# worldfnd/provekit

Hardware: AMD Instinct MI355X
Metric: proofs/sec (noir-r1cs prove hot path, WHIR commit + sumcheck + folding rounds) (higher is better)
Workload: dtype u32x8 (BN254-Fr, 256-bit Montgomery integers); 1 GPU; poseidon-rounds size class: m=21, m_0=20, satisfiable synthetic R1CS (786429 constraints, 1048571 witnesses, a constant term in half of the rows of A and B), batch-2 WHIR commit + zk-sumcheck + 4-round WHIR opening, queries [109, 28, 16, 11]/9, pow_bits [19.0, 16.0, 16.0, 18.0]/11.0 (WhirConfig::new derivation, security 128, ConjectureList), blinding WHIR n=8 queries [122]/31, Skyscraper-sponge tr; launcher=single process

## Files before the change

provekit_amd/_lib.py:

```python
from __future__ import annotations

import ctypes as C
import os

_HERE = os.path.dirname(os.path.abspath(__file__))
LIB_PATH = os.environ.get("PK_LIB_PATH") or os.path.join(_HERE, "lib", "libprovekit_hip.so")

PK_OK = 0
PK_LEAF_MAJOR = 0
PK_COL_MAJOR = 1

_ERR_NAMES = {-1: "PK_ERR_BAD_ARG", -2: "PK_ERR_OOM", -3: "PK_ERR_HIP", -4: "PK_ERR_RCCL", -5: "PK_ERR_NO_DEVICE", -6: "PK_ERR_UNSATISFIED"}


class ProveKitHipError(RuntimeError):
    def __init__(self, code, msg):
        super().__init__(f"{_ERR_NAMES.get(code, code)}: {msg}")
        self.code = code


def _load():
    if not os.path.exists(LIB_PATH):
        raise ImportError(
            f"{LIB_PATH} is missing: build it with `python -c 'import __graft_entry__ as g; g.build()'` "
# ... 125 lines not shown
}


class WhirConfigStruct(C.Structure):
    _fields_ = [("n_vars", C.c_uint), ("batch_size", C.c_uint), ("folding_factor", C.c_uint), ("starting_log_inv_rate", C.c_uint),
                ("n_rounds", C.c_uint), ("num_queries", C.c_uint * 16), ("ood_samples", C.c_uint * 16), ("pow_bits", C.c_double * 16),
                ("final_queries", C.c_uint), ("final_pow_bits", C.c_double), ("commitment_ood_samples", C.c_uint),
                ("final_folding_pow_bits", C.c_double)]


class SparseMatrixStruct(C.Structure):
    _fields_ = [("new_row_indices", vp), ("col_indices", vp), ("values", vp), ("nnz", sz)]

SELFTEST_SIGNATURES = {
    "pk_selftest_set_host_tail": (C.c_int, [vp, C.c_uint]),
    "pk_selftest_eq_suffix_tables": (C.c_int, [vp, vp, C.c_uint, vp]),
    "pk_selftest_sumcheck_cubic_spliteq": (C.c_int, [vp, vp, vp, vp, vp, C.c_uint, C.c_uint, vp, vp, vp]),
    "pk_selftest_sumcheck_quadratic_claim": (C.c_int, [vp, vp, vp, sz, vp, vp, vp, vp, vp]),
    "pk_selftest_keccak_tag": (C.c_int, [vp, sz, vp]),
    "pk_selftest_permute": (C.c_int, [vp, vp]),
    "pk_selftest_arith": (C.c_int, [C.c_int, vp, vp, vp, sz]),
    "pk_selftest_chacha": (C.c_int, [vp, C.c_uint64, C.c_uint32, C.c_uint32, C.c_int, vp]),
    "pk_selftest_random_fe": (C.c_int, [vp, vp, C.c_uint32, vp, sz]),
    "pk_selftest_dft": (C.c_int, [vp, vp, vp, C.c_int, C.c_int, sz]),
    "pk_selftest_pre_load": (C.c_int, [vp, vp, vp, C.c_int, C.c_int, sz]),
    "pk_selftest_set_hook": (C.c_int, [C.c_int, C.c_long]),
}

for _name, (_res, _args) in list(SIGNATURES.items()) + list(SELFTEST_SIGNATURES.items()):
    if _name in SELFTEST_SIGNATURES and os.environ.get("PK_LIB_PATH") and not hasattr(lib, _name):
# ... 5 lines not shown
```

provekit_amd/csrc/ctx.hip:

```cpp
#include "internal.hpp"
#include "fe29.hpp"

#include <sys/prctl.h>
#include <time.h>

#include <atomic>

using namespace pk;

#define PK_MAX_DEVICES 64
static std::atomic<int> g_poll_wait[PK_MAX_DEVICES];
static std::atomic<long> g_test_hooks[pk::PK_HOOK_COUNT];
static std::atomic<int> g_runtime_wait[PK_MAX_DEVICES];
static const bool g_runtime_wait_init = [] {
    for (auto& w : g_runtime_wait) w.store(-1, std::memory_order_relaxed);
    return true;
}();

namespace pk {
long test_hook(int which) { return which >= 0 && which < PK_HOOK_COUNT ? g_test_hooks[which].load(std::memory_order_relaxed) : 0; }
hipError_t wait_stream(int device, hipStream_t stream) {
    if (device < 0 || device >= PK_MAX_DEVICES || !g_poll_wait[device].load(std::memory_order_relaxed)) return hipStreamSynchronize(stream);
    long slack = -1;
    hipError_t e;
// ... 246 lines not shown
}

int pk_ctx_set_latency_mode(pk_ctx* ctx, int on) {
    if (!ctx) return PK_ERR_BAD_ARG;
    ctx->latency_mode = on != 0;
    return PK_OK;
}

int pk_selftest_set_host_tail(pk_ctx* ctx, unsigned log2_len) {
    if (!ctx) return PK_ERR_BAD_ARG;
    if (log2_len > PK_HOST_TAIL_MAX_LOG2) return set_err(ctx, PK_ERR_BAD_ARG, "bad argument: host tail threshold is 0 (off) or 1 .. %d", PK_HOST_TAIL_MAX_LOG2);
    ctx->host_tail_log2 = log2_len;
    return PK_OK;
}

}

namespace pk {
int ensure_scratch(pk_ctx* ctx, size_t bytes) {
    if (ctx->scratch_bytes >= bytes) return PK_OK;
    if (ctx->d_scratch) {
        PK_WAIT(ctx);
        PK_HIP(ctx, hipFree(ctx->d_scratch));
        ctx->d_scratch = nullptr;
        ctx->scratch_bytes = 0;
    }
    size_t sz = bytes < (1u << 20) ? (1u << 20) : bytes;
    PK_HIP(ctx, hipMalloc(&ctx->d_scratch, sz));
    ctx->scratch_bytes = sz;
    ctx->red_armed = ctx->pow_armed = false;
// ... 83 lines not shown
```

provekit_amd/csrc/ctx.hpp:

```cpp
#pragma once
#include <hip/hip_runtime.h>

#include <cstdarg>
#include <cstdio>
#include <cstring>
#include <map>
#include <string>
#include <vector>

#include "../../include/provekit_hip.h"

struct pk_prof_rec {
    const char* name;
    hipEvent_t e0, e1;
};

struct pk_comm;

#ifndef PK_HOST_TAIL_DEFAULT_LOG2
#define PK_HOST_TAIL_DEFAULT_LOG2 10
#endif
#define PK_HOST_TAIL_MAX_LOG2 11

struct pk_ctx {
    int device = 0;
    pk_comm* comm = nullptr;
    bool prof_on = false;
    std::vector<pk_prof_rec> prof;
    std::vector<hipEvent_t> ev_pool;
    hipStream_t own_stream = nullptr;
    hipStream_t stream = nullptr;
    hipEvent_t ev_start = nullptr, ev_stop = nullptr;
    int hash_version = 2;
    int num_cus = 256;
    char err[512] = {0};
    int err_code = 0;
    void* d_scratch = nullptr;
    size_t scratch_bytes = 0;
    void* h_pinned = nullptr;
    size_t pinned_bytes = 0;
    std::map<unsigned long long, void*> tables;
    unsigned red_seq = 0;
    bool latency_mode = false;
    unsigned gate_seq = 0;
    unsigned host_tail_log2 = PK_HOST_TAIL_DEFAULT_LOG2;
    void* d_ws = nullptr;
    void* d_ztab = nullptr;
    size_t ws_bytes = 0;
    char* h_mail = nullptr;
    size_t mail_bytes = 0, mail_off = 0;
    bool pow_armed = false;
    bool red_armed = false;
    bool red_across = false;
    void* d_xred = nullptr;
    const void* red_scales = nullptr;
};
#define PK_XRED_OWN_BYTES 2048

#define PK_PIN_ROOT 2048
#define PK_PIN_POW 2112
// ... 96 lines not shown
```

provekit_amd/csrc/prover.hip:

```cpp
#include <unistd.h>

#include <algorithm>
#include <chrono>
#include <cstdlib>
#include <string>
#include <vector>

#include "host_tail.hpp"
#include "internal.hpp"
#include "shard_map.hpp"
#include "prover_transcript.hpp"

using namespace pk;

struct pk_scheme {
    const pk_r1cs* r1cs = nullptr;
    size_t num_constraints = 0, num_witnesses = 0;
    unsigned m = 0, m_0 = 0;
    unsigned nb = 0;
    pk_whir_config whir_witness{}, whir_hiding{};
    char* arena = nullptr;
    size_t arena_bytes = 0;
    std::string domain_separator;
    char* noir_witness = nullptr;
// ... 137 lines not shown
    }
    for (int i = 0; i < 4; i++) out[i] = c[i];
}

std::vector<uint64_t> stir_queries(Transcript& T, size_t domain_size, unsigned fold, unsigned num_queries) {
    std::vector<uint8_t> raw(stir_query_bytes(domain_size, fold) * num_queries);
    T.challenge_bytes(raw.data(), raw.size());
    return stir_indexes(raw.data(), domain_size, fold, num_queries);
}

int pow_round(pk_ctx* ctx, Transcript& T, double bits) {
    if (bits <= 0.0) return PK_OK;
    uint8_t challenge[POW_CHALLENGE_BYTES], be[POW_NONCE_BYTES];
    T.challenge_bytes(challenge, sizeof challenge);
    uint64_t nonce = 0;
    const int rc = pow_solve_x(ctx, challenge, bits, &nonce, comm_world(ctx) > 1);
    nonce_to_bytes(nonce, be);
    T.add_bytes(be, sizeof be);
    return rc;
}

struct Commitment {
    unsigned n_vars = 0, batch = 0;
    fe* polys[4] = {};
    fe* evals[4] = {};
    fe* leaves = nullptr;
    fe* nodes = nullptr;
    size_t rows = 0, width = 0;
    pk_commit_layout layout{};
    std::vector<fe> ood_points;
    std::vector<fe> ood_answers;
    fe beta;
};

int emit_opening_hints(pk_ctx* ctx, Transcript& T, const Commitment& C, const std::vector<uint64_t>& idx) {
    const size_t k = idx.size(), width = C.width;
    const unsigned logn = ilog2(C.rows);
    const size_t plen = logn ? logn - 1 : 0;
    std::vector<uint64_t> leaves(4 * k * width), sib(4 * (k ? k : 1)), paths(4 * (k * plen ? k * plen : 1));
    CK(open_raw(ctx, U(C.leaves), U(C.nodes), C.rows, width, C.layout, idx.data(), k, 1, leaves.data(), sib.data(), paths.data()));
    const auto ser0 = std::chrono::steady_clock::now();
    std::vector<uint8_t> buf;
    put_u64(buf, k);
    for (size_t q = 0; q < k; q++) put_vec(buf, (const fe*)(leaves.data() + 4 * q * width), width, false);
    T.hint(buf.data(), buf.size());
    size_t len = 0;
    pk_multipath_serialize(idx.data(), k, plen, sib.data(), paths.data(), nullptr, 0, &len);
    std::vector<uint8_t> mp(len ? len : 1);
    CK(pk_multipath_serialize(idx.data(), k, plen, sib.data(), paths.data(), mp.data(), len, &len));
    T.hint(mp.data(), len);
    T.hint_seconds += std::chrono::duration<double>(std::chrono::steady_clock::now() - ser0).count();
    return PK_OK;
}

int whir_commit_compute(pk_ctx* ctx, Arena& A, unsigned n_vars, unsigned log_inv_rate, unsigned fold, fe* const* polys, unsigned batch,
                        Commitment& C) {
    C.n_vars = n_vars;
    C.batch = batch;
    C.rows = (size_t)1 << (n_vars + log_inv_rate - fold);
    C.width = (size_t)batch << fold;
    for (unsigned b = 0; b < batch; b++) C.polys[b] = polys[b];
    ALLOC(leaves, C.rows * C.width / shard_factor(ctx, C.rows));
    ALLOC(nodes, 2 * C.rows);
    C.leaves = leaves;
    C.nodes = nodes;
    CK(ensure_ws(ctx, commit_scratch_fes(ctx, C.rows, C.width) * 32));
    const uint64_t* ptrs[4];
    for (unsigned b = 0; b < batch; b++) ptrs[b] = U(polys[b]);
    return commit_into(ctx, ptrs, batch, n_vars, log_inv_rate, fold, U(leaves), U(nodes), (uint64_t*)ctx->d_ws, &C.layout);
}
int whir_commit_transcript(pk_ctx* ctx, const pk_whir_config& cfg, const fe& root, Transcript& T, Commitment& C) {
    const unsigned batch = C.batch;
    fe* const* polys = C.polys;
    T.add_canon(root);
    C.ood_points.resize(cfg.commitment_ood_samples);
    T.challenge_scalars(C.ood_points.data(), C.ood_points.size());
    C.ood_answers.resize((size_t)batch * C.ood_points.size());
    for (size_t j = 0; j < C.ood_points.size(); j++) {
        for (unsigned b = 0; b < batch; b += 2) {
            const unsigned np = batch - b >= 2 ? 2 : 1;
            fe ans[2];
            CK(eval_univariate_multi_x(ctx, polys + b, np, (size_t)1 << cfg.n_vars, C.ood_points[j], ans));
            for (unsigned q = 0; q < np; q++) C.ood_answers[(b + q) * C.ood_points.size() + j] = ans[q];
        }
    }
    for (unsigned b = 0; b < batch; b++) T.add_scalars(&C.ood_answers[b * C.ood_points.size()], C.ood_points.size());
    C.beta = batch > 1 ? T.challenge_scalar() : fe_one();
    return PK_OK;
}

bool whir_sharded(const pk_ctx* ctx, unsigned n_vars) {
    const size_t G = (size_t)comm_world(ctx);
    return G > 1 && (((size_t)1 << n_vars) / G) >= 2 * SHARD_MIN_LOCAL;
}
size_t in_block(size_t stored, size_t off, size_t len) {
    const size_t hi = stored < off + len ? stored : off + len;
    return hi > off ? hi - off : 0;
// ... 64 lines not shown

struct WhirProver {
    pk_ctx* ctx;
    Arena& A;
    const pk_whir_config& cfg;
    const Commitment& C;
    Transcript& T;
    const unsigned n, k, G, lgG, rank;
    bool sharded;
    const size_t B0, off0;
    fe* d_c = nullptr;
    fe* bp[2] = {};
    fe* bw[2] = {};
    fe* gathered[4] = {};
    bool host = false;
    std::vector<fe> hp, hw;
    const fe* h_weight = nullptr;
    int cur = 0;
    size_t len;
    std::vector<fe> rs;
    fe claim;
    bool have_claim = false;
    std::vector<fe> all_r;

    WhirProver(pk_ctx* c, Arena& a, const pk_whir_config& cf, const Commitment& com, Transcript& t)
        : ctx(c), A(a), cfg(cf), C(com), T(t), n(cf.n_vars), k(cf.folding_factor), G((unsigned)comm_world(c)), lgG(ilog2(G)),
          rank((unsigned)comm_rank(c)), sharded(whir_sharded(c, n)), B0(sharded ? ((size_t)1 << n) / G : (size_t)1 << n),
          off0(sharded ? (size_t)rank * B0 : 0), len(B0) {}

    int batch_combine(fe* dst, fe* const* x, size_t from, size_t cnt) {
        if (C.batch == 1) return pk_memcpy_d2d(ctx, dst, x[0] + from, 32 * cnt);
// ... 135 lines not shown
        return PK_OK;
    }
    int maybe_gather() { return sharded && len <= SHARD_MIN_LOCAL ? gather(gathered[0], gathered[1], gathered[2], gathered[3]) : PK_OK; }

    int start(fe* const* d_weights, const size_t* weight_len, unsigned n_weights, const fe* weight_sums, const fe* h_evals, const fe* h_w) {
        const size_t N = (size_t)1 << n;
        if (h_evals) {
            PK_REQUIRE(ctx, !sharded && C.batch == 2 && n_weights <= 1 && (!n_weights || (h_w && weight_len[0] <= N)),
                       "an opening that starts on the host: batch 2, one weight");
            host = true;
            h_weight = h_w;
            hp.resize(N);
            hw.resize(N);
            host_tail::lincomb2(hp.data(), h_evals, C.beta, h_evals + N, N);
        }
        ALLOC(dc, N);
        d_c = dc;
        ALLOC(p0, B0);
        ALLOC(p1, B0 / 2 ? B0 / 2 : 1);
        ALLOC(w0, B0);
        ALLOC(w1, B0 / 2 ? B0 / 2 : 1);
        bp[0] = p0; bp[1] = p1; bw[0] = w0; bw[1] = w1;
        bool have_evals = true;
        for (unsigned b = 0; b < C.batch; b++) have_evals = have_evals && C.evals[b] != nullptr;
        const bool pair = have_evals && C.batch == 2;
        const bool rows3 = rows_at_equal_stride3(d_weights, weight_len, n_weights);
        const size_t tail = host_tail_len(ctx);
        const bool fused = !host && !(tail && !sharded && B0 <= tail) && pair && !sharded && B0 >= 2 && k >= 1 && (rows3 || n_weights == 1) && weight_len[0] <= B0;
        if (fused || host) {
            h_store(first.beta, C.beta);
            CK(lincomb2(ctx, U(d_c), U(C.polys[0]), first.beta, U(C.polys[1]), N));
        } else if (pair) {
            uint64_t s[4];
            h_store(s, C.beta);
            CK(lincomb2_pair(ctx, U(d_c), U(C.polys[0]), U(C.polys[1]), N, U(p0), U(C.evals[0] + off0), U(C.evals[1] + off0), B0, s));
        } else {
            CK(batch_combine(d_c, C.polys, 0, N));
        }
        if (host) {
        } else if (have_evals) {
            if (!pair) CK(batch_combine(p0, C.evals, off0, B0));
        } else if (!sharded) {
            CK(pk_to_evals_into(ctx, U(d_c), U(p0), n));
        } else {
// ... 48 lines not shown
                gathered[q] = buf;
            }
        }
        CK(sumcheck_rounds(k));
        return maybe_gather();
    }

    int rounds() {
        const Commitment* prev = &C;
        Commitment com;
        unsigned nv = n, log_inv_rate = cfg.starting_log_inv_rate;
        size_t domain_size = (size_t)1 << (n + log_inv_rate);
        fe exp_gen = folded_domain_generator(n + log_inv_rate, k);
        for (unsigned r = 0; r < cfg.n_rounds; r++) {
            const unsigned nv2 = nv - k;
            ALLOC(d_c2, (size_t)1 << nv2);
            CK(pk_fold_coeffs(ctx, U(d_c), nv, (const uint64_t*)rs.data(), k, U(d_c2)));
            d_c = d_c2;
            nv = nv2;
            log_inv_rate += k - 1;
            Commitment next;
            CK(whir_commit_compute(ctx, A, nv, log_inv_rate, k, &d_c, 1, next));
            fe root;
            CK(read_root(ctx, U(next.nodes), next.rows, (uint64_t*)root.v));
            T.add_canon(root);
            std::vector<fe> zs(cfg.ood_samples[r]);
            T.challenge_scalars(zs.data(), zs.size());
            std::vector<fe> ood_ans(zs.size());
            for (size_t j = 0; j < zs.size(); j++) CK(eval_univariate_x(ctx, d_c, (size_t)1 << nv, zs[j], ood_ans[j]));
            T.add_scalars(ood_ans.data(), ood_ans.size());
            CK(pow_round(ctx, T, cfg.pow_bits[r]));
            const std::vector<uint64_t> idx = stir_queries(T, domain_size, k, cfg.num_queries[r]);
            CK(emit_opening_hints(ctx, T, *prev, idx));
            const fe gamma = T.challenge_scalar();
            for (uint64_t i : idx) zs.push_back(h_pow(exp_gen, i));
            fe g;
            CK(maybe_to_host());
            CK(eq_weights(bw[cur], nv, zs, gamma, 0, &g, !host && !sharded && len >= 2 && k >= 1));
            have_claim = false;
            CK(sumcheck_rounds(k));
            CK(maybe_gather());
            com = next;
            prev = &com;
            domain_size /= 2;
            exp_gen = h_mul(exp_gen, exp_gen);
        }
        return final_round(*prev, nv, domain_size);
    }

    int final_round(const Commitment& prev, unsigned nv, size_t domain_size) {
        if (sharded) {
            const size_t cap = len * G;
            ALLOC(fp0, cap);
            ALLOC(fp1, cap / 2 ? cap / 2 : 1);
            ALLOC(fw0, cap);
            ALLOC(fw1, cap / 2 ? cap / 2 : 1);
            CK(gather(fp0, fp1, fw0, fw1));
        }
        const unsigned nv2 = nv - k;
        ALLOC(d_final, (size_t)1 << nv2);
        CK(pk_fold_coeffs(ctx, U(d_c), nv, (const uint64_t*)rs.data(), k, U(d_final)));
        std::vector<fe> fin((size_t)1 << nv2);
        CK(pk_memcpy_d2h(ctx, fin.data(), d_final, 32 * fin.size()));
        T.add_scalars(fin.data(), fin.size());
        CK(pow_round(ctx, T, cfg.final_pow_bits));
        const std::vector<uint64_t> idx = stir_queries(T, domain_size, k, cfg.final_queries);
        CK(emit_opening_hints(ctx, T, prev, idx));
        CK(sumcheck_rounds(nv2));
        return pow_round(ctx, T, cfg.final_folding_pow_bits);
    }

    int deferred_hint(fe* const* d_weights, const size_t* weight_len, unsigned n_weights) {
        if (!n_weights) return PK_OK;
        std::vector<fe> point(all_r.rbegin(), all_r.rend());
        const bool sh = whir_sharded(ctx, n);
        std::vector<fe> evals(n_weights);
        const bool rows3 = rows_at_equal_stride3(d_weights, weight_len, n_weights);
        if (h_weight) {
// ... 33 lines not shown
        return PK_OK;
    }
};
int whir_prove(pk_ctx* ctx, Arena& A, const pk_whir_config& cfg, const Commitment& C, fe* const* d_weights, const size_t* weight_len,
               unsigned n_weights, const fe* weight_sums, Transcript& T, const fe* h_evals = nullptr, const fe* h_weight = nullptr) {
    WhirProver P(ctx, A, cfg, C, T);
    CK(P.start(d_weights, weight_len, n_weights, weight_sums, h_evals, h_weight));
    CK(P.rounds());
    return P.deferred_hint(d_weights, weight_len, n_weights);
}

struct BatchCommit {
    Commitment com;
    fe* f_evals = nullptr;
    fe* g_evals = nullptr;
};
int batch_commit_compute(pk_ctx* ctx, Arena& A, unsigned m, const pk_whir_config& cfg, const fe* d_evals, size_t n_evals, const RngKey& key,
                         u32 stream_mask, u32 stream_g, BatchCommit& out) {
    const size_t half = (size_t)1 << (m - 1), N = 2 * half;
    ALLOC(f, N);
    ALLOC(g, N);
    ALLOC(fe_, N);
    ALLOC(ge_, N);
    if (comm_world(ctx) <= 1) {
        CK(to_coeffs_generated(ctx, m, U(d_evals), n_evals, key, stream_mask, stream_g, U(f), U(g), U(fe_), U(ge_)));
    } else {
        CK(pk_memset_zero(ctx, f, 32 * half));
        CK(pk_memcpy_d2d(ctx, f, d_evals, 32 * n_evals));
        {
            ProfScope prof(ctx, "random_fe");
// ... 79 lines not shown
    fe row_sums[6];
    const bool timing = getenv("PK_PROVE_TIMING") != nullptr;
    std::chrono::steady_clock::time_point t_lap = std::chrono::steady_clock::now();

    Proof(pk_ctx* c, pk_scheme* sc, const fe* w, size_t nw, const RngKey& k)
        : ctx(c), s(sc), d_witness(w), n_witness(nw), key(k), A{sc->arena, sc->arena_bytes}, T(sc->domain_separator), G((unsigned)comm_world(c)),
          lgG(ilog2(G)), rank((unsigned)comm_rank(c)), st_sharded(whir_sharded(c, sc->m)), blk(((size_t)1 << sc->m) / (st_sharded ? G : 1)),
          blk_lo(st_sharded ? (size_t)rank * blk : 0), aux(c), g_univ(4 * (size_t)sc->m_0) {}

    int init() {
        if (!ctx->latency_mode || G != 1) return PK_OK;
        CK(side.open(ctx, s));
        aux = side.c;
        return PK_OK;
    }
    pk_ctx* rows_ctx() const { return n_witness ? aux : ctx; }
    int relay(pk_ctx* c, int rc, const char* what) {
        if (!rc || c == ctx) return rc;
        return set_err(ctx, rc, "%s on the side stream: %s", what, pk_last_error(c));
    }
    void lap(const char* what) {
        if (!timing) return;
        (void)wait_ctx(ctx);
        const auto t = std::chrono::steady_clock::now();
        fprintf(stderr, "[pk_prove] %-28s %8.3f ms (sponge: %u permutes, %.3f ms; hint serialisation so far %.3f ms)\n", what,
                1e3 * std::chrono::duration<double>(t - t_lap).count(), T.permutes(), 1e3 * T.permute_seconds, 1e3 * T.hint_seconds);
        t_lap = t;
    }

    int commit_witness();
// ... 8 lines not shown
int blinding_compute(pk_ctx* ctx, Proof& P) {
    Arena& A = P.A;
    const size_t NB = (size_t)1 << P.s->nb, n = P.g_univ.size();
    ALLOC(d_blind, NB);
    CK(pk_memset_zero(ctx, d_blind, 32 * NB));
    CK(random_fe(ctx, U(d_blind), n, P.key, RNG_BLIND));
    if (ctx == P.ctx) {
        CK(pk_memcpy_d2h(ctx, P.g_univ.data(), d_blind, 32 * n));
    } else {
        CK(mail_alloc(ctx, 32 * n, (void**)&P.h_univ));
        PK_HIP(ctx, hipMemcpyAsync(P.h_univ, d_blind, 32 * n, hipMemcpyDeviceToHost, ctx->stream));
    }
    return batch_commit_compute(ctx, A, P.s->nb + 1, P.s->whir_hiding, d_blind, NB, P.key, RNG_MASK_B, RNG_G_B, P.B);
}

int external_rows(pk_ctx* ctx, Proof& P) {
    Arena& A = P.A;
    const size_t nw = P.n_witness;
    ALLOC(d_eq_alpha, (size_t)1 << P.s->m_0);
    ALLOC(rows, 3 * (nw ? nw : 1));
    P.rows = rows;
    CK(pk_eq_table(ctx, (const uint64_t*)P.alpha.data(), P.s->m_0, U(d_eq_alpha)));
    if (P.st_sharded) CK(external_row_range(ctx, P.s->r1cs, U(d_eq_alpha), P.blk_lo, std::min(nw, P.blk_lo + P.blk), U(rows)));
    else CK(pk_r1cs_external_row(ctx, P.s->r1cs, U(d_eq_alpha), U(rows)));
    if (ctx == P.ctx) return PK_OK;
    return dot_rows(ctx, U(rows), nw, 3, U(P.W.f_evals), U(P.W.g_evals), nw, nullptr, true);
}

int Proof::commit_witness() {
    CK(batch_commit_compute(ctx, A, s->m, s->whir_witness, d_witness, n_witness, key, RNG_MASK, RNG_G, W));
    if (aux != ctx) CK(relay(aux, blinding_compute(aux, *this), "blinding commitment"));
    fe root;
    CK(read_root(ctx, U(W.com.nodes), W.com.rows, (uint64_t*)root.v));
    return whir_commit_transcript(ctx, s->whir_witness, root, T, W.com);
}

int Proof::blinding_transcript() {
    fe root;
    CK(relay(aux, read_root(aux, U(B.com.nodes), B.com.rows, (uint64_t*)root.v), "blinding commitment"));
    if (h_univ) memcpy(g_univ.data(), h_univ, 32 * g_univ.size());
    return whir_commit_transcript(ctx, s->whir_hiding, root, T, B.com);
}

void zk_round_message(const uint64_t out[12], const fe gp[4], const fe& rho, const fe& saved, fe c[4]) {
    const fe half = h_half();
    c[0] = h_add(h_load(out), h_mul(rho, gp[0]));
    const fe g_m1 = h_sub(h_add(h_sub(gp[0], gp[1]), gp[2]), gp[3]);
    const fe at_m1 = h_add(h_load(out + 4), h_mul(rho, g_m1));
    c[2] = h_mul(half, h_sub(h_sub(h_sub(h_add(saved, at_m1), c[0]), c[0]), c[0]));
    c[3] = h_add(h_load(out + 8), h_mul(rho, gp[3]));
    c[1] = h_sub(h_sub(h_sub(h_sub(saved, c[0]), c[0]), c[3]), c[2]);
}

int Proof::zk_sumcheck() {
// ... 3 lines not shown
    const size_t M0 = (size_t)1 << m_0;
    const bool sharded = G > 1 && M0 / G >= 2 * SHARD_MIN_LOCAL;
    const size_t length = sharded ? M0 / G : M0;
    ALLOC(d_a, length);
    ALLOC(d_b, length);
    ALLOC(d_cc, length);
    ALLOC(d_eq, length);
    if (sharded) {
        CK(witness_bounds_strided(ctx, s->r1cs, U(d_witness), m_0, G, rank, U(d_a), U(d_b), U(d_cc)));
        const fe sc = eq_bits(&r[m_0 - lgG], lgG, rank);
        CK(pk_eq_accumulate(ctx, U(d_eq), m_0 - lgG, (const uint64_t*)r.data(), (const uint64_t*)&sc, 1, 1));
    } else {
        CK(pk_r1cs_witness_bounds(ctx, s->r1cs, U(d_witness), m_0, U(d_a), U(d_b), U(d_cc)));
        CK(eq_suffix_tables(ctx, (const uint64_t*)r.data(), m_0, U(d_eq)));
    }
    if (aux == ctx) CK(blinding_compute(ctx, *this));
    CK(blinding_transcript());
    lap("bounds+eq+blinding commit");
    fe* z[4] = {d_a, d_b, d_cc, d_eq};
    return zk_rounds(z, length, sharded, sharded ? nullptr : r.data());
}

struct ZkRounds {
    Proof& pf;
    pk_ctx* ctx;
    fe** z;
    size_t len;
    bool sharded;
    const fe* r;
    const size_t M;
    fe rho, saved;
// ... 82 lines not shown
    }
    alpha.reserve(m_0);
    return sumcheck_round_loop(ctx, T, m_0, ctx->latency_mode && G == 1 && m_0 >= 2, R);
}

int Proof::prove_blinding() {
    if (rows_ctx() != ctx) CK(relay(aux, external_rows(aux, *this), "external rows"));
    const size_t nbw = 4 * (size_t)s->m_0;
    std::vector<fe> wv(nbw);
    for (size_t i = 0; i < s->m_0; i++) {
        wv[4 * i] = fe_one();
        wv[4 * i + 1] = alpha[i];
        wv[4 * i + 2] = h_mul(alpha[i], alpha[i]);
        wv[4 * i + 3] = h_mul(wv[4 * i + 2], alpha[i]);
    }
    ALLOC(d_bw, nbw);
    uint64_t fg[8];
    const size_t NB2 = (size_t)2 << s->nb, tail = host_tail_len(ctx);
    std::vector<fe> h_evals;
    if (tail && NB2 <= tail) {
        h_evals.resize(2 * NB2);
        const uint64_t* src[2] = {U(B.f_evals), U(B.g_evals)};
        const size_t cnt[2] = {NB2, NB2};
        CK(tables_to_host(ctx, src, cnt, 2, U(h_evals.data())));
        host_tail::dot2(wv.data(), h_evals.data(), h_evals.data() + NB2, nbw, fg);
    } else {
        CK(pk_memcpy_h2d(ctx, d_bw, wv.data(), 32 * nbw));
        CK(pk_dot2(ctx, U(d_bw), U(B.f_evals), U(B.g_evals), nbw, fg));
    }
    const fe sums[2] = {h_load(fg), h_load(fg + 4)};
    T.add_scalars(sums, 2);
    fe* wts[1] = {d_bw};
    return whir_prove(ctx, A, s->whir_hiding, B.com, wts, &nbw, 1, sums, T, h_evals.empty() ? nullptr : h_evals.data(), h_evals.empty() ? nullptr : wv.data());
}

int Proof::witness_statement() {
    pk_ctx* rc = rows_ctx();
    if (rc == ctx) CK(external_rows(ctx, *this));
    Across ac(ctx, st_sharded);
    CK(ac.rc);
    uint64_t o[24] = {};
    if (rc != ctx) {
        CK(relay(rc, sync_stream(rc), "external rows"));
        memcpy(o, rc->h_pinned, 32 * 6);
    } else if (st_sharded || n_witness) {
        CK(dot_rows(ctx, U(rows + blk_lo), n_witness, 3, U(W.f_evals + blk_lo), U(W.g_evals + blk_lo), in_block(n_witness, blk_lo, blk), o));
    }
    fe fsum[3], gsum[3];
// ... 170 lines not shown

int pk_scheme_set_io_pattern(pk_ctx* ctx, pk_scheme* s, const uint8_t* pattern, size_t n) {
    PK_ENTER(ctx);
    PK_REQUIRE(ctx, s, "null pointer");
    if (!pattern || !n) {
        s->domain_separator = whir_r1cs_io_pattern(s->m_0, s->whir_witness, s->whir_hiding);
        return PK_OK;
    }
    const std::string theirs((const char*)pattern, n);
    const std::string bad = io_pattern_mismatch(theirs, s->m_0, s->whir_witness, s->whir_hiding);
    if (!bad.empty()) return set_err(ctx, PK_ERR_IO_PATTERN, "%s", bad.c_str());
    s->domain_separator = theirs;
    return PK_OK;
}

}
```

provekit_amd/runtime.py:

```python
from __future__ import annotations

import ctypes as C

import numpy as np

from . import _lib
from ._lib import ProveKitHipError, lib


class DeviceBuffer:

    def __init__(self, ctx: "Context", nbytes: int):
        self.ctx = ctx
        self.nbytes = int(nbytes)
        p = C.c_void_p()
        ctx._check(lib.pk_malloc(ctx.handle, self.nbytes, C.byref(p)))
        self.ptr = p.value

    def free(self):
        if self.ptr is not None and self.ctx.handle is not None:
            lib.pk_free(self.ctx.handle, self.ptr)
        self.ptr = None

    def __del__(self):
# ... 48 lines not shown
    def comm_unique_id() -> bytes:
        buf = (C.c_uint8 * 128)()
        rc = lib.pk_comm_unique_id(buf)
        if rc != 0:
            raise ProveKitHipError(rc, "pk_comm_unique_id failed (librccl not loadable?)")
        return bytes(buf)

    def comm_init_rank(self, unique_id: bytes, world: int, rank: int):
        self._check(lib.pk_comm_init_rank(self.handle, (C.c_uint8 * 128).from_buffer_copy(unique_id), world, rank))

    def set_latency_mode(self, on: bool = True):
        self._check(lib.pk_ctx_set_latency_mode(self.handle, 1 if on else 0))

    def set_host_tail(self, log2_len: int):
        self._check(lib.pk_selftest_set_host_tail(self.handle, log2_len))

    def comm_info(self):
        r, w, k = C.c_int(), C.c_int(), C.c_int()
        self._check(lib.pk_comm_info(self.handle, C.byref(r), C.byref(w), C.byref(k)))
        return r.value, w.value, k.value

    def comm_destroy(self):
        self._check(lib.pk_comm_destroy(self.handle))

    @staticmethod
    def set_host_wait(device: int, mode):
        code = {False: 0, True: 1, "spin": 0, "block": 1, "poll": 2}[mode]
        rc = lib.pk_device_set_host_wait(device, code)
        if rc != 0:
            raise ProveKitHipError(rc, "pk_device_set_host_wait failed")
# ... 97 lines not shown
```

Measured before the change: 297.0 proofs/s.

## Run small blinding WHIR commit, folds and low-bit PoW grinding on the host

Adds a CPU implementation of the WHIR pieces used on tiny polynomials: NTT-based RS encoding, Merkle hashing, openings, coefficient folding, Horner evaluation and proof-of-work grinding. When the host-tail threshold allows it, the blinding commitment (n=8) and later small rounds are computed on the host instead of launching many small GPU kernels. PoW challenges of at most 4 bits are also ground on the CPU. This is meant to remove kernel-launch and synchronisation latency on tiny work, at the cost of serial CPU Poseidon/Skyscraper hashing, which could be slower if the sizes are larger than expected.

```diff
diff --git a/provekit_amd/_lib.py b/provekit_amd/_lib.py
--- a/provekit_amd/_lib.py
+++ b/provekit_amd/_lib.py
@@ -163,6 +163,9 @@
 
 SELFTEST_SIGNATURES = {
     "pk_selftest_set_host_tail": (C.c_int, [vp, C.c_uint]),
+    "pk_selftest_set_host_pow": (C.c_int, [vp, C.c_uint]),
+    "pk_selftest_host_commit": (C.c_int, [C.c_int, vp, C.c_uint, C.c_uint, C.c_uint, C.c_uint, vp, vp]),
+    "pk_selftest_host_pow": (C.c_int, [vp, C.c_double, C.POINTER(C.c_uint64)]),
     "pk_selftest_eq_suffix_tables": (C.c_int, [vp, vp, C.c_uint, vp]),
     "pk_selftest_sumcheck_cubic_spliteq": (C.c_int, [vp, vp, vp, vp, vp, C.c_uint, C.c_uint, vp, vp, vp]),
     "pk_selftest_sumcheck_quadratic_claim": (C.c_int, [vp, vp, vp, sz, vp, vp, vp, vp, vp]),
diff --git a/provekit_amd/csrc/ctx.hip b/provekit_amd/csrc/ctx.hip
--- a/provekit_amd/csrc/ctx.hip
+++ b/provekit_amd/csrc/ctx.hip
@@ -284,6 +284,13 @@
     return PK_OK;
 }
 
+int pk_selftest_set_host_pow(pk_ctx* ctx, unsigned max_bits) {
+    if (!ctx) return PK_ERR_BAD_ARG;
+    if (max_bits > PK_HOST_POW_CEILING) return set_err(ctx, PK_ERR_BAD_ARG, "bad argument: host grinder bound is 0 (off) or 1 .. %d bits", PK_HOST_POW_CEILING);
+    ctx->host_pow_max_bits = max_bits;
+    return PK_OK;
+}
+
 }
 
 namespace pk {
diff --git a/provekit_amd/csrc/ctx.hpp b/provekit_amd/csrc/ctx.hpp
--- a/provekit_amd/csrc/ctx.hpp
+++ b/provekit_amd/csrc/ctx.hpp
@@ -21,6 +21,10 @@
 #define PK_HOST_TAIL_DEFAULT_LOG2 10
 #endif
 #define PK_HOST_TAIL_MAX_LOG2 11
+#ifndef PK_HOST_POW_MAX_BITS
+#define PK_HOST_POW_MAX_BITS 4
+#endif
+#define PK_HOST_POW_CEILING 8
 
 struct pk_ctx {
     int device = 0;
@@ -44,6 +48,7 @@
     bool latency_mode = false;
     unsigned gate_seq = 0;
     unsigned host_tail_log2 = PK_HOST_TAIL_DEFAULT_LOG2;
+    unsigned host_pow_max_bits = PK_HOST_POW_MAX_BITS;
     void* d_ws = nullptr;
     void* d_ztab = nullptr;
     size_t ws_bytes = 0;
diff --git a/provekit_amd/csrc/host_whir.hpp b/provekit_amd/csrc/host_whir.hpp
--- /dev/null
+++ b/provekit_amd/csrc/host_whir.hpp
@@ -0,0 +1,122 @@
+#pragma once
+#include <vector>
+
+#include "host_tail.hpp"
+
+namespace pk {
+namespace host_whir {
+
+using host_tail::mul;
+
+inline void ntt(fe* x, unsigned log_n) {
+    const size_t n = (size_t)1 << log_n;
+    for (size_t i = 0; i < n; i++) {
+        size_t r = 0;
+        for (unsigned b = 0; b < log_n; b++) r |= ((i >> b) & 1) << (log_n - 1 - b);
+        if (r > i) std::swap(x[i], x[r]);
+    }
+    std::vector<fe> w(n / 2 ? n / 2 : 1);
+    w[0] = fe_one();
+    const fe gen = domain_generator(log_n);
+    for (size_t e = 1; e < n / 2; e++) w[e] = mul(w[e - 1], gen);
+    for (size_t len = 2; len <= n; len <<= 1) {
+        const size_t step = n / len;
+        for (size_t base = 0; base < n; base += len)
+            for (size_t t = 0; t < len / 2; t++) {
+                const fe a = x[base + t], b = mul(x[base + t + len / 2], w[t * step]);
+                x[base + t] = h_add(a, b);
+                x[base + t + len / 2] = h_sub(a, b);
+            }
+    }
+}
+inline void rs_encode(const fe* const* polys, unsigned batch, unsigned n_vars, unsigned log_inv_rate, unsigned fold, fe* leaves) {
+    const unsigned log_rows = n_vars + log_inv_rate - fold;
+    const size_t rows = (size_t)1 << log_rows, fw = (size_t)1 << fold, L = (size_t)1 << (n_vars - fold);
+    for (unsigned b = 0; b < batch; b++)
+        for (size_t j = 0; j < fw; j++) {
+            fe* col = leaves + (b * fw + j) * rows;
+            for (size_t t = 0; t < rows; t++) col[t] = t < L ? polys[b][fw * t + j] : fe_zero();
+            ntt(col, log_rows);
+        }
+}
+
+inline fe compress(int version, const fe& l, const fe& r) {
+    if (version == 2) {
+        fe a = fe_reduce_any(l), b = fe_reduce_any(r);
+        const fe l0 = a;
+        sky_permute_host(a, b);
+        return fe_add(a, l0);
+    }
+    return pack29(compress29<1, true>(unpack_reduce29(l), unpack_reduce29(r)));
+}
+inline void leaf_hash(int version, const fe* leaves, size_t rows, size_t width, fe* digests) {
+    for (size_t i = 0; i < rows; i++) {
+        fe h = h_to_canon(leaves[i]);
+        for (size_t j = 1; j < width; j++) h = compress(version, h, h_to_canon(leaves[j * rows + i]));
+        digests[i] = h;
+    }
+}
+inline void merkle_inner(int version, fe* nodes, size_t rows) {
+    for (size_t i = rows - 1; i >= 1; i--) nodes[i] = compress(version, nodes[2 * i], nodes[2 * i + 1]);
+    nodes[0] = fe_zero();
+}
+inline void commit(int version, const fe* const* polys, unsigned batch, unsigned n_vars, unsigned log_inv_rate, unsigned fold, fe* leaves, fe* nodes) {
+    const size_t rows = (size_t)1 << (n_vars + log_inv_rate - fold), width = (size_t)batch << fold;
+    rs_encode(polys, batch, n_vars, log_inv_rate, fold, leaves);
+    leaf_hash(version, leaves, rows, width, nodes + rows);
+    merkle_inner(version, nodes, rows);
+}
+
+inline void open(const fe* leaves, const fe* nodes, size_t rows, size_t width, const uint64_t* idx, size_t k, fe* out_leaves, fe* out_sib, fe* out_path) {
+    unsigned logn = 0;
+    while (((size_t)1 << logn) < rows) logn++;
+    const unsigned plen = logn ? logn - 1 : 0;
+    for (size_t q = 0; q < k; q++) {
+        const size_t i = (size_t)idx[q], node = rows + i;
+        for (size_t j = 0; j < width; j++) out_leaves[q * width + j] = h_to_canon(leaves[j * rows + i]);
+        if (logn) out_sib[q] = nodes[node ^ 1];
+        for (unsigned d = 0; d < plen; d++) out_path[q * plen + d] = nodes[(node >> (logn - (d + 1))) ^ 1];
+    }
+}
+
+inline void fold_coeffs(const fe* c, unsigned n_vars, const fe* r, unsigned k, fe* out) {
+    const size_t fw = (size_t)1 << k, n_out = (size_t)1 << (n_vars - k);
+    std::vector<fe> w(fw);
+    w[0] = fe_one();
+    for (unsigned b = 0; b < k; b++)
+        for (size_t j = 0; j < ((size_t)1 << b); j++) w[j | ((size_t)1 << b)] = mul(w[j], r[b]);
+    for (size_t t = 0; t < n_out; t++) {
+        fe acc = c[t * fw];
+        for (size_t j = 1; j < fw; j++) acc = h_add(acc, mul(c[t * fw + j], w[j]));
+        out[t] = acc;
+    }
+}
+
+inline fe horner(const fe* c, size_t n, const fe& z) {
+    fe acc = fe_zero();
+    for (size_t i = n; i-- > 0;) acc = h_add(mul(acc, z), c[i]);
+    return acc;
+}
+
+inline bool pow_valid(const fe& challenge_reduced, const uint64_t thr[4], uint64_t nonce) {
+    fe a = challenge_reduced, b = fe_zero();
+    b.v[0] = (u32)nonce;
+    b.v[1] = (u32)(nonce >> 32);
+    sky_permute_host(a, b);
+    const fe h = fe_add(a, challenge_reduced);
+    fe t;
+    memcpy(t.v, thr, 32);
+    return fe_lt(h, t);
+}
+inline uint64_t pow_grind(const uint8_t challenge[POW_CHALLENGE_BYTES], double bits) {
+    if (bits <= 0.0) return 0;
+    uint64_t thr[4];
+    pow_threshold(bits + 0.01, thr);
+    const fe ch = fe_reduce_any(load_raw(challenge));
+    uint64_t nonce = 0;
+    while (!pow_valid(ch, thr, nonce)) nonce++;
+    return nonce;
+}
+
+}
+}
diff --git a/provekit_amd/csrc/host_whir_asan_main.cpp b/provekit_amd/csrc/host_whir_asan_main.cpp
--- /dev/null
+++ b/provekit_amd/csrc/host_whir_asan_main.cpp
@@ -0,0 +1,212 @@
+#include <cstdio>
+#include <cstdlib>
+
+#include "host_whir.hpp"
+
+namespace {
+
+using namespace pk;
+namespace hw = pk::host_whir;
+
+uint64_t rng_state = 0x9e3779b97f4a7c15ULL;
+uint64_t next_u64() {
+    rng_state ^= rng_state << 13;
+    rng_state ^= rng_state >> 7;
+    rng_state ^= rng_state << 17;
+    return rng_state;
+}
+fe p_minus_1() {
+    fe r;
+    for (int i = 0; i < 8; i++) r.v[i] = kPlimb(i);
+    r.v[0] -= 1;
+    return r;
+}
+fe random_fe() {
+    fe r;
+    for (int i = 0; i < 8; i += 2) {
+        const uint64_t x = next_u64();
+        r.v[i] = (u32)x;
+        r.v[i + 1] = (u32)(x >> 32);
+    }
+    return fe_reduce_any(r);
+}
+fe draw(int kind) {
+    if (kind == 4) kind = (int)(next_u64() & 3);
+    return kind == 0 ? fe_zero() : kind == 1 ? fe_one() : kind == 2 ? p_minus_1() : random_fe();
+}
+std::vector<fe> table(size_t n, int kind) {
+    std::vector<fe> t(n);
+    for (auto& x : t) x = draw(kind);
+    return t;
+}
+
+int failures = 0;
+void expect(const fe& got, const fe& want, const char* what, size_t a, int b, int c) {
+    if (fe_eq(got, want)) return;
+    if (failures < 20) printf("MISMATCH %s %zu %d %d\n", what, a, b, c);
+    failures++;
+}
+
+fe horner_naive(const fe* c, size_t n, const fe& z) {
+    fe acc = fe_zero(), zp = fe_one();
+    for (size_t i = 0; i < n; i++) {
+        acc = h_add(acc, h_mul(c[i], zp));
+        zp = h_mul(zp, z);
+    }
+    return acc;
+}
+fe root_naive(int version, const std::vector<fe>& digests, size_t lo, size_t n) {
+    if (n == 1) return digests[lo];
+    return hw::compress(version, root_naive(version, digests, lo, n / 2), root_naive(version, digests, lo + n / 2, n / 2));
+}
+
+struct Shape {
+    unsigned n_vars, log_inv_rate, fold, batch;
+};
+const Shape SHAPES[] = {{4, 1, 4, 1}, {4, 1, 4, 2}, {5, 1, 4, 1}, {5, 1, 4, 2}, {6, 1, 4, 1}, {6, 1, 4, 2}, {8, 1, 4, 1}, {8, 1, 4, 2}, {4, 4, 4, 1}};
+
+void check_commit_and_open() {
+    for (const Shape& s : SHAPES)
+        for (int kind = 0; kind < 5; kind++)
+            for (int version = 1; version <= 2; version++) {
+                if (version == 1 && kind != 4) continue;
+                const size_t N = (size_t)1 << s.n_vars, fw = (size_t)1 << s.fold, width = (size_t)s.batch << s.fold;
+                const unsigned log_rows = s.n_vars + s.log_inv_rate - s.fold;
+                const size_t rows = (size_t)1 << log_rows;
+                std::vector<std::vector<fe>> polys;
+                const fe* ptrs[2];
+                for (unsigned b = 0; b < s.batch; b++) {
+                    polys.push_back(table(N, kind));
+                    ptrs[b] = polys[b].data();
+                }
+                std::vector<fe> leaves(rows * width), nodes(2 * rows);
+                hw::commit(version, ptrs, s.batch, s.n_vars, s.log_inv_rate, s.fold, leaves.data(), nodes.data());
+                const fe w = domain_generator(log_rows);
+                fe wi = fe_one();
+                std::vector<fe> digests(rows);
+                for (size_t i = 0; i < rows; i++, wi = h_mul(wi, w)) {
+                    fe h = fe_zero();
+                    for (size_t col = 0; col < width; col++) {
+                        const size_t b = col / fw, j = col % fw;
+                        std::vector<fe> sub(N / fw);
+                        for (size_t t = 0; t < N / fw; t++) sub[t] = polys[b][fw * t + j];
+                        const fe want = horner_naive(sub.data(), sub.size(), wi);
+                        expect(leaves[col * rows + i], want, "codeword", rows, kind, (int)col);
+                        h = col ? hw::compress(version, h, h_to_canon(want)) : h_to_canon(want);
+                    }
+                    digests[i] = h;
+                    expect(nodes[rows + i], h, "leaf digest", rows, kind, (int)i);
+                }
+                expect(nodes[1], root_naive(version, digests, 0, rows), "root", rows, kind, version);
+                expect(nodes[0], fe_zero(), "heap slot 0", rows, kind, version);
+                for (size_t i = 1; i < rows; i++) expect(nodes[i], hw::compress(version, nodes[2 * i], nodes[2 * i + 1]), "inner node", rows, kind, (int)i);
+                std::vector<uint64_t> all(rows), rep;
+                for (size_t i = 0; i < rows; i++) all[i] = i;
+                for (size_t q = 0; q < 7; q++) rep.push_back(next_u64() % rows), rep.push_back(rep.back());
+                for (const std::vector<uint64_t>& idx : {all, rep}) {
+                    const size_t k = idx.size(), plen = log_rows ? log_rows - 1 : 0;
+                    std::vector<fe> ol(k * width), os(log_rows ? k : 0), op(k * plen);
+                    hw::open(leaves.data(), nodes.data(), rows, width, idx.data(), k, ol.data(), os.data(), op.data());
+                    for (size_t q = 0; q < k; q++) {
+                        fe h = ol[q * width];
+                        for (size_t j = 0; j < width; j++) expect(ol[q * width + j], h_to_canon(leaves[j * rows + idx[q]]), "opened leaf", rows, kind, (int)q);
+                        for (size_t j = 1; j < width; j++) h = hw::compress(version, h, ol[q * width + j]);
+                        uint64_t i = idx[q];
+                        h = (i & 1) ? hw::compress(version, os[q], h) : hw::compress(version, h, os[q]);
+                        i >>= 1;
+                        for (size_t d = plen; d-- > 0;) {
+                            const fe& node = op[q * plen + d];
+                            h = (i & 1) ? hw::compress(version, node, h) : hw::compress(version, h, node);
+                            i >>= 1;
+                        }
+                        expect(h, nodes[1], "opening reaches the root", rows, kind, (int)q);
+                    }
+                }
+            }
+    {
+        const std::vector<fe> c = table(16, 3);
+        const fe* ptrs[1] = {c.data()};
+        std::vector<fe> leaves(16), nodes(2);
+        hw::commit(2, ptrs, 1, 4, 0, 4, leaves.data(), nodes.data());
+        fe h = h_to_canon(c[0]);
+        for (size_t j = 1; j < 16; j++) h = hw::compress(2, h, h_to_canon(c[j]));
+        expect(nodes[1], h, "one leaf", 1, 3, 0);
+    }
+    for (int kind = 0; kind < 4; kind++)
+        for (int k2 = 0; k2 < 4; k2++) {
+            const fe l = h_to_canon(draw(kind)), r = h_to_canon(draw(k2));
+            expect(hw::compress(2, l, r), pack29(compress29<2, true>(unpack_reduce29(l), unpack_reduce29(r))), "compress v2", 0, kind, k2);
+        }
+    printf("commitments and openings ok\n");
+}
+
+void check_fold_and_horner() {
+    for (unsigned n : {4u, 5u, 8u})
+        for (unsigned k : {1u, 4u})
+            for (int kind = 0; kind < 5; kind++) {
+                const size_t N = (size_t)1 << n, fw = (size_t)1 << k;
+                const std::vector<fe> c = table(N, kind), r = table(k, kind == 0 ? 3 : kind);
+                std::vector<fe> out(N >> k);
+                hw::fold_coeffs(c.data(), n, r.data(), k, out.data());
+                for (size_t t = 0; t < (N >> k); t++) {
+                    fe want = fe_zero();
+                    for (size_t j = 0; j < fw; j++) {
+                        fe w = fe_one();
+                        for (unsigned b = 0; b < k; b++)
+                            if ((j >> b) & 1) w = h_mul(w, r[b]);
+                        want = h_add(want, h_mul(c[t * fw + j], w));
+                    }
+                    expect(out[t], want, "fold_coeffs", N, kind, (int)t);
+                }
+                const fe z = draw(kind);
+                expect(hw::horner(c.data(), N, z), horner_naive(c.data(), N, z), "horner", N, kind, 0);
+            }
+    expect(hw::horner(nullptr, 0, fe_one()), fe_zero(), "horner of nothing", 0, 0, 0);
+    printf("folds and evaluations ok\n");
+}
+
+void check_grinder() {
+    for (double bits : {0.0, 1.0, 4.0, 6.0, 8.0})
+        for (int c = 0; c < 3; c++) {
+            uint8_t ch[32];
+            for (int i = 0; i < 32; i += 8) {
+                const uint64_t x = c == 0 && i == 24 ? ~0ull : next_u64();
+                memcpy(ch + i, &x, 8);
+            }
+            const uint64_t got = hw::pow_grind(ch, bits);
+            if (bits == 0.0) {
+                if (got != 0) printf("MISMATCH grinder at 0 bits\n"), failures++;
+                continue;
+            }
+            uint64_t thr[4];
+            pow_threshold(bits + 0.01, thr);
+            fe t;
+            memcpy(t.v, thr, 32);
+            for (uint64_t nonce = 0; nonce <= got; nonce++) {
+                fe nn = fe_zero();
+                nn.v[0] = (u32)nonce;
+                nn.v[1] = (u32)(nonce >> 32);
+                const bool ok = fe_lt(hw::compress(2, load_raw(ch), nn), t);
+                if (ok != (nonce == got)) {
+                    printf("MISMATCH grinder bits %.0f nonce %llu of %llu\n", bits, (unsigned long long)nonce, (unsigned long long)got);
+                    failures++;
+                    break;
+                }
+            }
+        }
+    printf("grinder ok\n");
+}
+
+}
+
+int main() {
+    check_commit_and_open();
+    check_fold_and_horner();
+    check_grinder();
+    if (failures) {
+        printf("%d differences\n", failures);
+        return 1;
+    }
+    printf("host whir ok\n");
+    return 0;
+}
diff --git a/provekit_amd/csrc/prover.hip b/provekit_amd/csrc/prover.hip
--- a/provekit_amd/csrc/prover.hip
+++ b/provekit_amd/csrc/prover.hip
@@ -3,10 +3,12 @@
 #include <algorithm>
 #include <chrono>
 #include <cstdlib>
+#include <memory>
 #include <string>
 #include <vector>
 
 #include "host_tail.hpp"
+#include "host_whir.hpp"
 #include "internal.hpp"
 #include "shard_map.hpp"
 #include "prover_transcript.hpp"
@@ -175,7 +177,9 @@
     uint8_t challenge[POW_CHALLENGE_BYTES], be[POW_NONCE_BYTES];
     T.challenge_bytes(challenge, sizeof challenge);
     uint64_t nonce = 0;
-    const int rc = pow_solve_x(ctx, challenge, bits, &nonce, comm_world(ctx) > 1);
+    int rc = PK_OK;
+    if (host_tail_len(ctx) && bits <= (double)ctx->host_pow_max_bits) nonce = host_whir::pow_grind(challenge, bits);
+    else rc = pow_solve_x(ctx, challenge, bits, &nonce, comm_world(ctx) > 1);
     nonce_to_bytes(nonce, be);
     T.add_bytes(be, sizeof be);
     return rc;
@@ -188,6 +192,8 @@
     fe* leaves = nullptr;
     fe* nodes = nullptr;
     size_t rows = 0, width = 0;
+    bool host = false;
+    std::shared_ptr<std::vector<fe>> mem;
     pk_commit_layout layout{};
     std::vector<fe> ood_points;
     std::vector<fe> ood_answers;
@@ -199,7 +205,8 @@
     const unsigned logn = ilog2(C.rows);
     const size_t plen = logn ? logn - 1 : 0;
     std::vector<uint64_t> leaves(4 * k * width), sib(4 * (k ? k : 1)), paths(4 * (k * plen ? k * plen : 1));
-    CK(open_raw(ctx, U(C.leaves), U(C.nodes), C.rows, width, C.layout, idx.data(), k, 1, leaves.data(), sib.data(), paths.data()));
+    if (C.host) host_whir::open(C.leaves, C.nodes, C.rows, width, idx.data(), k, (fe*)leaves.data(), (fe*)sib.data(), (fe*)paths.data());
+    else CK(open_raw(ctx, U(C.leaves), U(C.nodes), C.rows, width, C.layout, idx.data(), k, 1, leaves.data(), sib.data(), paths.data()));
     const auto ser0 = std::chrono::steady_clock::now();
     std::vector<uint8_t> buf;
     put_u64(buf, k);
@@ -230,6 +237,19 @@
     for (unsigned b = 0; b < batch; b++) ptrs[b] = U(polys[b]);
     return commit_into(ctx, ptrs, batch, n_vars, log_inv_rate, fold, U(leaves), U(nodes), (uint64_t*)ctx->d_ws, &C.layout);
 }
+void whir_commit_host(const pk_ctx* ctx, unsigned n_vars, unsigned log_inv_rate, unsigned fold, fe* const* polys, unsigned batch, Commitment& C) {
+    C.n_vars = n_vars;
+    C.batch = batch;
+    C.rows = (size_t)1 << (n_vars + log_inv_rate - fold);
+    C.width = (size_t)batch << fold;
+    for (unsigned b = 0; b < batch; b++) C.polys[b] = polys[b];
+    C.host = true;
+    C.mem = std::make_shared<std::vector<fe>>(C.rows * C.width + 2 * C.rows);
+    C.leaves = C.mem->data();
+    C.nodes = C.leaves + C.rows * C.width;
+    C.layout = pk_commit_layout{1, 0, PK_LEAVES_MONTGOMERY};
+    host_whir::commit(ctx->hash_version, polys, batch, n_vars, log_inv_rate, fold, C.leaves, C.nodes);
+}
 int whir_commit_transcript(pk_ctx* ctx, const pk_whir_config& cfg, const fe& root, Transcript& T, Commitment& C) {
     const unsigned batch = C.batch;
     fe* const* polys = C.polys;
@@ -241,7 +261,8 @@
         for (unsigned b = 0; b < batch; b += 2) {
             const unsigned np = batch - b >= 2 ? 2 : 1;
             fe ans[2];
-            CK(eval_univariate_multi_x(ctx, polys + b, np, (size_t)1 << cfg.n_vars, C.ood_points[j], ans));
+            if (C.host) for (unsigned q = 0; q < np; q++) ans[q] = host_whir::horner(polys[b + q], (size_t)1 << cfg.n_vars, C.ood_points[j]);
+            else CK(eval_univariate_multi_x(ctx, polys + b, np, (size_t)1 << cfg.n_vars, C.ood_points[j], ans));
             for (unsigned q = 0; q < np; q++) C.ood_answers[(b + q) * C.ood_points.size() + j] = ans[q];
         }
     }
@@ -336,7 +357,7 @@
     fe* bw[2] = {};
     fe* gathered[4] = {};
     bool host = false;
-    std::vector<fe> hp, hw;
+    std::vector<fe> hp, hw, hc;
     const fe* h_weight = nullptr;
     int cur = 0;
     size_t len;
@@ -502,20 +523,29 @@
             hw.resize(N);
             host_tail::lincomb2(hp.data(), h_evals, C.beta, h_evals + N, N);
         }
-        ALLOC(dc, N);
-        d_c = dc;
-        ALLOC(p0, B0);
-        ALLOC(p1, B0 / 2 ? B0 / 2 : 1);
-        ALLOC(w0, B0);
-        ALLOC(w1, B0 / 2 ? B0 / 2 : 1);
-        bp[0] = p0; bp[1] = p1; bw[0] = w0; bw[1] = w1;
+        fe *p0 = nullptr, *w0 = nullptr;
+        if (C.host) {
+            PK_REQUIRE(ctx, host, "a host commitment is opened from the host's tables");
+            hc.resize(N);
+            host_tail::lincomb2(hc.data(), C.polys[0], C.beta, C.polys[1], N);
+        } else {
+            ALLOC(dc, N);
+            d_c = dc;
+            ALLOC(p0_, B0);
+            ALLOC(p1, B0 / 2 ? B0 / 2 : 1);
+            ALLOC(w0_, B0);
+            ALLOC(w1, B0 / 2 ? B0 / 2 : 1);
+            p0 = p0_, w0 = w0_;
+            bp[0] = p0; bp[1] = p1; bw[0] = w0; bw[1] = w1;
+        }
         bool have_evals = true;
         for (unsigned b = 0; b < C.batch; b++) have_evals = have_evals && C.evals[b] != nullptr;
         const bool pair = have_evals && C.batch == 2;
         const bool rows3 = rows_at_equal_stride3(d_weights, weight_len, n_weights);
         const size_t tail = host_tail_len(ctx);
         const bool fused = !host && !(tail && !sharded && B0 <= tail) && pair && !sharded && B0 >= 2 && k >= 1 && (rows3 || n_weights == 1) && weight_len[0] <= B0;
-        if (fused || host) {
+        if (C.host) {
+        } else if (fused || host) {
             h_store(first.beta, C.beta);
             CK(lincomb2(ctx, U(d_c), U(C.polys[0]), first.beta, U(C.polys[1]), N));
         } else if (pair) {
@@ -594,20 +624,35 @@
         fe exp_gen = folded_domain_generator(n + log_inv_rate, k);
         for (unsigned r = 0; r < cfg.n_rounds; r++) {
             const unsigned nv2 = nv - k;
-            ALLOC(d_c2, (size_t)1 << nv2);
-            CK(pk_fold_coeffs(ctx, U(d_c), nv, (const uint64_t*)rs.data(), k, U(d_c2)));
-            d_c = d_c2;
+            if (C.host) {
+                std::vector<fe> hc2((size_t)1 << nv2);
+                host_whir::fold_coeffs(hc.data(), nv, rs.data(), k, hc2.data());
+                hc.swap(hc2);
+                d_c = hc.data();
+            } else {
+                ALLOC(d_c2, (size_t)1 << nv2);
+                CK(pk_fold_coeffs(ctx, U(d_c), nv, (const uint64_t*)rs.data(), k, U(d_c2)));
+                d_c = d_c2;
+            }
             nv = nv2;
             log_inv_rate += k - 1;
             Commitment next;
-            CK(whir_commit_compute(ctx, A, nv, log_inv_rate, k, &d_c, 1, next));
             fe root;
-            CK(read_root(ctx, U(next.nodes), next.rows, (uint64_t*)root.v));
+            if (C.host) {
+                whir_commit_host(ctx, nv, log_inv_rate, k, &d_c, 1, next);
+                root = next.nodes[1];
+            } else {
+                CK(whir_commit_compute(ctx, A, nv, log_inv_rate, k, &d_c, 1, next));
+                CK(read_root(ctx, U(next.nodes), next.rows, (uint64_t*)root.v));
+            }
             T.add_canon(root);
             std::vector<fe> zs(cfg.ood_samples[r]);
             T.challenge_scalars(zs.data(), zs.size());
             std::vector<fe> ood_ans(zs.size());
-            for (size_t j = 0; j < zs.size(); j++) CK(eval_univariate_x(ctx, d_c, (size_t)1 << nv, zs[j], ood_ans[j]));
+            for (size_t j = 0; j < zs.size(); j++) {
+                if (next.host) ood_ans[j] = host_whir::horner(d_c, (size_t)1 << nv, zs[j]);
+                else CK(eval_univariate_x(ctx, d_c, (size_t)1 << nv, zs[j], ood_ans[j]));
+            }
             T.add_scalars(ood_ans.data(), ood_ans.size());
             CK(pow_round(ctx, T, cfg.pow_bits[r]));
             const std::vector<uint64_t> idx = stir_queries(T, domain_size, k, cfg.num_queries[r]);
@@ -638,10 +683,14 @@
             CK(gather(fp0, fp1, fw0, fw1));
         }
         const unsigned nv2 = nv - k;
-        ALLOC(d_final, (size_t)1 << nv2);
-        CK(pk_fold_coeffs(ctx, U(d_c), nv, (const uint64_t*)rs.data(), k, U(d_final)));
         std::vector<fe> fin((size_t)1 << nv2);
-        CK(pk_memcpy_d2h(ctx, fin.data(), d_final, 32 * fin.size()));
+        if (C.host) {
+            host_whir::fold_coeffs(hc.data(), nv, rs.data(), k, fin.data());
+        } else {
+            ALLOC(d_final, (size_t)1 << nv2);
+            CK(pk_fold_coeffs(ctx, U(d_c), nv, (const uint64_t*)rs.data(), k, U(d_final)));
+            CK(pk_memcpy_d2h(ctx, fin.data(), d_final, 32 * fin.size()));
+        }
         T.add_scalars(fin.data(), fin.size());
         CK(pow_round(ctx, T, cfg.final_pow_bits));
         const std::vector<uint64_t> idx = stir_queries(T, domain_size, k, cfg.final_queries);
@@ -705,6 +754,7 @@
     Commitment com;
     fe* f_evals = nullptr;
     fe* g_evals = nullptr;
+    std::vector<fe> h_tables;
 };
 int batch_commit_compute(pk_ctx* ctx, Arena& A, unsigned m, const pk_whir_config& cfg, const fe* d_evals, size_t n_evals, const RngKey& key,
                          u32 stream_mask, u32 stream_g, BatchCommit& out) {
@@ -814,6 +864,7 @@
         aux = side.c;
         return PK_OK;
     }
+    bool blinding_on_host() const { return host_tail_len(ctx) && ((size_t)2 << s->nb) <= host_tail_len(ctx); }
     pk_ctx* rows_ctx() const { return n_witness ? aux : ctx; }
     int relay(pk_ctx* c, int rc, const char* what) {
         if (!rc || c == ctx) return rc;
@@ -852,6 +903,38 @@
     return batch_commit_compute(ctx, A, P.s->nb + 1, P.s->whir_hiding, d_blind, NB, P.key, RNG_MASK_B, RNG_G_B, P.B);
 }
 
+int blinding_tables_to_host(pk_ctx* ctx, Proof& P) {
+    Arena& A = P.A;
+    const unsigned mb = P.s->nb + 1;
+    const size_t NB = (size_t)1 << P.s->nb, N = 2 * NB, n = P.g_univ.size();
+    ALLOC(d_blind, NB);
+    ALLOC(f, N);
+    ALLOC(g, N);
+    ALLOC(fc, N);
+    ALLOC(gc, N);
+    CK(pk_memset_zero(ctx, d_blind, 32 * NB));
+    CK(random_fe(ctx, U(d_blind), n, P.key, RNG_BLIND));
+    CK(to_coeffs_generated(ctx, mb, U(d_blind), NB, P.key, RNG_MASK_B, RNG_G_B, U(f), U(g), U(fc), U(gc)));
+    P.B.h_tables.resize(4 * N);
+    const uint64_t* src[4] = {U(f), U(g), U(fc), U(gc)};
+    const size_t cnt[4] = {N, N, N, N};
+    CK(tables_to_host(ctx, src, cnt, 4, U(P.B.h_tables.data())));
+    std::copy(P.B.h_tables.begin(), P.B.h_tables.begin() + n, P.g_univ.begin());
+    return PK_OK;
+}
+void blinding_commit_host(const pk_ctx* ctx, Proof& P) {
+    BatchCommit& out = P.B;
+    const pk_whir_config& cfg = P.s->whir_hiding;
+    const size_t N = (size_t)2 << P.s->nb;
+    fe *f = out.h_tables.data(), *g = f + N;
+    out.f_evals = f;
+    out.g_evals = g;
+    fe* polys[2] = {g + N, g + 2 * N};
+    whir_commit_host(ctx, cfg.n_vars, cfg.starting_log_inv_rate, cfg.folding_factor, polys, 2, out.com);
+    out.com.evals[0] = f;
+    out.com.evals[1] = g;
+}
+
 int external_rows(pk_ctx* ctx, Proof& P) {
     Arena& A = P.A;
     const size_t nw = P.n_witness;
@@ -866,8 +949,14 @@
 }
 
 int Proof::commit_witness() {
+    const bool hostb = blinding_on_host();
+    if (hostb) CK(blinding_tables_to_host(ctx, *this));
     CK(batch_commit_compute(ctx, A, s->m, s->whir_witness, d_witness, n_witness, key, RNG_MASK, RNG_G, W));
-    if (aux != ctx) CK(relay(aux, blinding_compute(aux, *this), "blinding commitment"));
+    if (hostb) {
+        blinding_commit_host(ctx, *this);
+    } else if (aux != ctx) {
+        CK(relay(aux, blinding_compute(aux, *this), "blinding commitment"));
+    }
     fe root;
     CK(read_root(ctx, U(W.com.nodes), W.com.rows, (uint64_t*)root.v));
     return whir_commit_transcript(ctx, s->whir_witness, root, T, W.com);
@@ -875,7 +964,8 @@
 
 int Proof::blinding_transcript() {
     fe root;
-    CK(relay(aux, read_root(aux, U(B.com.nodes), B.com.rows, (uint64_t*)root.v), "blinding commitment"));
+    if (B.com.host) root = B.com.nodes[1];
+    else CK(relay(aux, read_root(aux, U(B.com.nodes), B.com.rows, (uint64_t*)root.v), "blinding commitment"));
     if (h_univ) memcpy(g_univ.data(), h_univ, 32 * g_univ.size());
     return whir_commit_transcript(ctx, s->whir_hiding, root, T, B.com);
 }
@@ -909,7 +999,7 @@
         CK(pk_r1cs_witness_bounds(ctx, s->r1cs, U(d_witness), m_0, U(d_a), U(d_b), U(d_cc)));
         CK(eq_suffix_tables(ctx, (const uint64_t*)r.data(), m_0, U(d_eq)));
     }
-    if (aux == ctx) CK(blinding_compute(ctx, *this));
+    if (aux == ctx && !B.com.host) CK(blinding_compute(ctx, *this));
     CK(blinding_transcript());
     lap("bounds+eq+blinding commit");
     fe* z[4] = {d_a, d_b, d_cc, d_eq};
@@ -1022,24 +1112,29 @@
         wv[4 * i + 2] = h_mul(alpha[i], alpha[i]);
         wv[4 * i + 3] = h_mul(wv[4 * i + 2], alpha[i]);
     }
-    ALLOC(d_bw, nbw);
     uint64_t fg[8];
     const size_t NB2 = (size_t)2 << s->nb, tail = host_tail_len(ctx);
     std::vector<fe> h_evals;
-    if (tail && NB2 <= tail) {
+    fe* d_bw = nullptr;
+    if (B.com.host) {
+        host_tail::dot2(wv.data(), B.f_evals, B.g_evals, nbw, fg);
+    } else if (tail && NB2 <= tail) {
         h_evals.resize(2 * NB2);
         const uint64_t* src[2] = {U(B.f_evals), U(B.g_evals)};
         const size_t cnt[2] = {NB2, NB2};
         CK(tables_to_host(ctx, src, cnt, 2, U(h_evals.data())));
         host_tail::dot2(wv.data(), h_evals.data(), h_evals.data() + NB2, nbw, fg);
     } else {
+        ALLOC(bw_, nbw);
+        d_bw = bw_;
         CK(pk_memcpy_h2d(ctx, d_bw, wv.data(), 32 * nbw));
         CK(pk_dot2(ctx, U(d_bw), U(B.f_evals), U(B.g_evals), nbw, fg));
     }
     const fe sums[2] = {h_load(fg), h_load(fg + 4)};
     T.add_scalars(sums, 2);
     fe* wts[1] = {d_bw};
-    return whir_prove(ctx, A, s->whir_hiding, B.com, wts, &nbw, 1, sums, T, h_evals.empty() ? nullptr : h_evals.data(), h_evals.empty() ? nullptr : wv.data());
+    const fe* h_ev = B.com.host ? B.f_evals : h_evals.empty() ? nullptr : h_evals.data();
+    return whir_prove(ctx, A, s->whir_hiding, B.com, wts, &nbw, 1, sums, T, h_ev, h_ev ? wv.data() : nullptr);
 }
 
 int Proof::witness_statement() {
@@ -1240,4 +1335,21 @@
     return PK_OK;
 }
 
-}
+
+int pk_selftest_host_commit(int hash_version, const uint64_t* coeffs, unsigned batch, unsigned n_vars, unsigned log_inv_rate, unsigned fold,
+                            uint64_t* leaves_out, uint64_t* nodes_out) {
+    if (!coeffs || !leaves_out || !nodes_out || (hash_version != 1 && hash_version != 2) || batch < 1 || batch > 4 || fold > n_vars ||
+        n_vars + log_inv_rate - fold > PK_HOST_TAIL_MAX_LOG2)
+        return PK_ERR_BAD_ARG;
+    const fe* polys[4];
+    for (unsigned b = 0; b < batch; b++) polys[b] = (const fe*)coeffs + ((size_t)b << n_vars);
+    host_whir::commit(hash_version, polys, batch, n_vars, log_inv_rate, fold, (fe*)leaves_out, (fe*)nodes_out);
+    return PK_OK;
+}
+int pk_selftest_host_pow(const uint8_t challenge[32], double bits, uint64_t* nonce) {
+    if (!challenge || !nonce || !(bits >= 0.0 && bits <= (double)PK_HOST_POW_CEILING)) return PK_ERR_BAD_ARG;
+    *nonce = host_whir::pow_grind(challenge, bits);
+    return PK_OK;
+}
+
+}
diff --git a/provekit_amd/runtime.py b/provekit_amd/runtime.py
--- a/provekit_amd/runtime.py
+++ b/provekit_amd/runtime.py
@@ -86,6 +86,9 @@
 
     def set_host_tail(self, log2_len: int):
         self._check(lib.pk_selftest_set_host_tail(self.handle, log2_len))
+
+    def set_host_pow(self, max_bits: int):
+        self._check(lib.pk_selftest_set_host_pow(self.handle, max_bits))
 
     def comm_info(self):
         r, w, k = C.c_int(), C.c_int(), C.c_int()
```

Measured after the change: 304.5 proofs/s (median of 6 runs). 2.5% higher.
